# COMPiLELab/krylov_robustness

Hardware: AMD Instinct MI355X
Metric: trace(exp(A)) evals/sec + achieved HBM GB/s, n=1M nnz=10M, 1/2/4/8 GPU (higher is better)
Workload: dtype f64

## Files before the change

krylov_robustness_amd/csrc/kt_kernels.hip:

```cpp
#include <hip/hip_runtime.h>

#include "kt_launch.h"
#include "kt_wave.h"
#include <stdint.h>

#include <cstdlib>

#include <type_traits>

namespace kt {

__device__ __forceinline__ uint64_t sm64(uint64_t x) {
    uint64_t z = x + 0x9E3779B97F4A7C15ULL;
    z = (z ^ (z >> 30)) * 0xBF58476D1CE4E5B9ULL;
    z = (z ^ (z >> 27)) * 0x94D049BB133111EBULL;
    return z ^ (z >> 31);
}

template <int P, int VW> struct GeoW {
    static constexpr int VEC = VW;
    static constexpr int LPR = P / VEC;
    static constexpr int GPW = 64 / LPR;
};
template <int P> using Geo = GeoW<P, (P >= 2) ? 2 : 1>;
// ... 981 lines not shown
__global__ __launch_bounds__(256) void k_inf_norm(int n, int nc, const double* __restrict__ X,
                                                  int ldx, double* __restrict__ partial) {
    double mx = 0.0;
    for (int r = blockIdx.x * blockDim.x + threadIdx.x; r < n; r += gridDim.x * blockDim.x) {
        double s = 0.0;
        for (int c = 0; c < nc; ++c) s += fabs(X[(int64_t)r * ldx + c]);
        mx = fmax(mx, s);
    }
    for (int o = 32; o > 0; o >>= 1) mx = fmax(mx, kt::shfl_xor(mx, o));
    __shared__ double red[4];
    if ((threadIdx.x & 63) == 0) red[threadIdx.x >> 6] = mx;
    __syncthreads();
    if (threadIdx.x == 0) partial[blockIdx.x] = fmax(fmax(red[0], red[1]), fmax(red[2], red[3]));
}

__global__ __launch_bounds__(256) void k_normest1_y(int n, const double* __restrict__ Y,
                                                   const double* __restrict__ Sprev,
                                                   double* __restrict__ S,
                                                   double* __restrict__ partial) {
    double a = 0.0, d = 0.0;
    for (int r = blockIdx.x * blockDim.x + threadIdx.x; r < n; r += gridDim.x * blockDim.x) {
        const double y = Y[r];
        const double s = y < 0.0 ? -1.0 : 1.0;
        a += fabs(y);
        d = fma(Sprev[r], s, d);
        S[r] = s;
    }
    for (int o = 32; o > 0; o >>= 1) {
        a += kt::shfl_xor(a, o);
        d += kt::shfl_xor(d, o);
// ... 87 lines not shown
    if ((threadIdx.x & 63) == 0) red[threadIdx.x >> 6] = mx;
    __syncthreads();
    if (threadIdx.x == 0) {
        st->c1 = fmax(fmax(red[0], red[1]), fmax(red[2], red[3]));
        st->c1s[1] = st->c1;
        st->active = 1;
    }
    if (threadIdx.x < kTermSlots) {
        st->term_max[1][threadIdx.x][0] = 0ull;
        st->term_max[1][threadIdx.x][1] = 0ull;
    }
}

__global__ __launch_bounds__(256) void k_expmv_term(int n, int nc, double mu, double coef,
                                                    const double* __restrict__ Ab, double* __restrict__ b,
                                                    double* __restrict__ F, int ld,
                                                    double* __restrict__ partial,
                                                    const ExpmvState* __restrict__ st) {
    if (!st->active) return;
    double mb = 0.0, mf = 0.0;
    for (int r = blockIdx.x * blockDim.x + threadIdx.x; r < n; r += gridDim.x * blockDim.x) {
        double sb = 0.0, sf = 0.0;
        for (int c = 0; c < nc; ++c) {
            const int64_t o = (int64_t)r * ld + c;
            double t = Ab[o];
            if (mu != 0.0) t = fma(-mu, b[o], t);
            const double bn = fma(coef, t, 0.0);
            const double f = fma(1.0, bn, F[o]);
            b[o] = bn;
            F[o] = f;
            sb += fabs(bn);
            sf += fabs(f);
        }
        mb = fmax(mb, sb);
        mf = fmax(mf, sf);
    }
    for (int o = 32; o > 0; o >>= 1) {
        mb = fmax(mb, kt::shfl_xor(mb, o));
        mf = fmax(mf, kt::shfl_xor(mf, o));
    }
    __shared__ double red[2][4];
    if ((threadIdx.x & 63) == 0) {
        red[0][threadIdx.x >> 6] = mb;
        red[1][threadIdx.x >> 6] = mf;
    }
    __syncthreads();
    if (threadIdx.x == 0) {
        partial[blockIdx.x] = fmax(fmax(red[0][0], red[0][1]), fmax(red[0][2], red[0][3]));
        partial[gridDim.x + blockIdx.x] = fmax(fmax(red[1][0], red[1][1]), fmax(red[1][2], red[1][3]));
    }
}

template <int VEC>
__device__ __forceinline__ void expmv_row_prefetch(int row, int p0, int nc, int ld, double mu,
                                                   const double* __restrict__ bin,
                                                   const double* __restrict__ F, double* fo, double* bo) {
#pragma unroll
    for (int e = 0; e < VEC; ++e) {
        const int c = p0 + e;
        const int64_t o = (int64_t)row * ld + c;
        fo[e] = (c < nc) ? F[o] : 0.0;
        bo[e] = (c < nc && mu != 0.0) ? bin[o] : 0.0;
    }
}
template <int VEC, bool PADW = true>
__device__ __forceinline__ void expmv_row_update(int row, int p0, const double* s, const double* fo,
                                                 const double* bo, int nc, int ld, double mu, double coef,
                                                 double* __restrict__ bout, double* __restrict__ F,
                                                 double& sb, double& sf) {
#pragma unroll
    for (int e = 0; e < VEC; ++e) {
        const int c = p0 + e;
        const int64_t o = (int64_t)row * ld + c;
        if (c < nc) {
            double t = s[e];
            if (mu != 0.0) t = fma(-mu, bo[e], t);
            const double bn = fma(coef, t, 0.0);
            const double f = fma(1.0, bn, fo[e]);
            bout[o] = bn;
            F[o] = f;
            sb += fabs(bn);
            sf += fabs(f);
        } else if constexpr (PADW) {
            bout[o] = 0.0;
        }
    }
}

constexpr int kExpmvWaves = 4;
constexpr int kExpmvSplitBlocks = 1024;

template <int P, int FLAGS, bool SPLIT>
__global__ __launch_bounds__(64 * kExpmvWaves) void k_expmv_step(
    const int* __restrict__ rp, const int* __restrict__ ci, const double* __restrict__ va, int n,
    const int* __restrict__ long_rows, int n_long, const int* __restrict__ med_rows, int n_med,
    int nc, int ld, double mu, double coef, double tol, int k, const double* __restrict__ bin,
    double* __restrict__ bout, double* __restrict__ F, ExpmvState* st, int* hflag, int stage) {
    constexpr int WAVES = kExpmvWaves;
    using G = GeoW<P, (P >= 2) ? 2 : 1>;
    using GL = GeoW<P, (P >= 4) ? 4 : (P >= 2) ? 2 : 1>;
    __shared__ double red[2][WAVES];
    __shared__ double lred[WAVES][P];
    __shared__ int decide;
    const int lane = threadIdx.x & 63;
    const int wave = threadIdx.x >> 6;
    const int med_blocks = (n_med + WAVES - 1) / WAVES;
    const int kind = ((int)blockIdx.x < n_long) ? 2 : ((int)blockIdx.x < n_long + med_blocks) ? 1 : 0;
    if constexpr (SPLIT) {
        if (threadIdx.x == 0) decide = st->active;
        __syncthreads();
        if (!decide) return;
// ... 4 lines not shown
    if (!SPLIT && wave == 0 && k > 1) {
        pmb = st->term_max[(k - 1) % 3][lane][0];
        pmf = st->term_max[(k - 1) % 3][lane][1];
    }
    const int subL = lane % GL::LPR, grpL = lane / GL::LPR, p0L = subL * GL::VEC;
    const int sub = lane % G::LPR, grp = lane / G::LPR, p0 = sub * G::VEC;
    double sl[GL::VEC], s[G::VEC], fo[GL::VEC], bo[GL::VEC];
#pragma unroll
    for (int e = 0; e < GL::VEC; ++e) sl[e] = fo[e] = bo[e] = 0.0;
#pragma unroll
    for (int e = 0; e < G::VEC; ++e) s[e] = 0.0;
    int row = -1;
    bool mine = false;
    if (kind == 2) {
        row = long_rows[blockIdx.x];
        if (!SPLIT && wave == 0 && grpL == 0) expmv_row_prefetch<GL::VEC>(row, p0L, nc, ld, mu, bin, F, fo, bo);
        row_gather8<P, FLAGS, GL>(rp[row] + wave * GL::GPW + grpL, rp[row + 1], WAVES * GL::GPW, p0L, ci,
                                  va, bin, sl, ld);
    } else if (kind == 1) {
        const int mi = ((int)blockIdx.x - n_long) * WAVES + wave;
        if (mi < n_med) {
            row = med_rows[mi];
            if (!SPLIT && grpL == 0) expmv_row_prefetch<GL::VEC>(row, p0L, nc, ld, mu, bin, F, fo, bo);
            row_gather8<P, FLAGS, GL>(rp[row] + grpL, rp[row + 1], GL::GPW, p0L, ci, va, bin, sl, ld);
            mine = grpL == 0;
        }
    } else {
        row = (((int)blockIdx.x - n_long - med_blocks) * WAVES + wave) * G::GPW + grp;
        if (row < n) {
            const int beg = rp[row], end = rp[row + 1];
            if (end - beg <= kMedThresh) {
                if (!SPLIT) expmv_row_prefetch<G::VEC>(row, p0, nc, ld, mu, bin, F, fo, bo);
                row_gather8<P, FLAGS, G>(beg, end, 1, p0, ci, va, bin, s, ld);
                mine = true;
            }
        }
    }
    if (kind != 0) {
#pragma unroll
        for (int o = GL::LPR; o < 64; o <<= 1)
#pragma unroll
            for (int e = 0; e < GL::VEC; ++e) sl[e] += kt::shfl_xor(sl[e], o);
    }
    if (kind == 2 && grpL == 0)
#pragma unroll
        for (int e = 0; e < GL::VEC; ++e) lred[wave][p0L + e] = sl[e];
    if constexpr (!SPLIT) {
// ... 20 lines not shown
    __syncthreads();
    if (!decide) return;
    } else {
        __syncthreads();
    }
    if (blockIdx.x == 0) {
        if (threadIdx.x == 0) st->mv += 1;
        if (!SPLIT && threadIdx.x < kTermSlots) {
            st->term_max[(k + 1) % 3][threadIdx.x][0] = 0ull;
            st->term_max[(k + 1) % 3][threadIdx.x][1] = 0ull;
        }
    }
    double sb = 0.0, sf = 0.0;
    if (kind == 0) {
        if (mine) {
            if constexpr (SPLIT) expmv_row_prefetch<G::VEC>(row, p0, nc, ld, mu, bin, F, fo, bo);
            expmv_row_update<G::VEC>(row, p0, s, fo, bo, nc, ld, mu, coef, bout, F, sb, sf);
        }
#pragma unroll
        for (int o = 1; o < G::LPR; o <<= 1) {
            sb += kt::shfl_xor(sb, o);
            sf += kt::shfl_xor(sf, o);
        }
    } else {
        if (kind == 2 && wave == 0 && grpL == 0) {
#pragma unroll
            for (int e = 0; e < GL::VEC; ++e)
            {
                double t = lred[0][p0L + e];
#pragma unroll
                for (int w = 1; w < WAVES; ++w) t += lred[w][p0L + e];
                sl[e] = t;
            }
            mine = true;
        }
        if (mine) {
            if constexpr (SPLIT) expmv_row_prefetch<GL::VEC>(row, p0L, nc, ld, mu, bin, F, fo, bo);
            expmv_row_update<GL::VEC>(row, p0L, sl, fo, bo, nc, ld, mu, coef, bout, F, sb, sf);
        }
#pragma unroll
        for (int o = 1; o < GL::LPR; o <<= 1) {
            sb += kt::shfl_xor(sb, o);
            sf += kt::shfl_xor(sf, o);
        }
    }
    double mb = sb, mf = sf;
#pragma unroll
    for (int o = 32; o > 0; o >>= 1) {
        mb = fmax(mb, kt::shfl_xor(mb, o));
        mf = fmax(mf, kt::shfl_xor(mf, o));
    }
    if (lane == 0) {
        red[0][wave] = mb;
// ... 9 lines not shown
        }
        unsigned long long* slot = st->term_max[k % 3][blockIdx.x % kTermSlots];
        __hip_atomic_fetch_max(slot, (unsigned long long)__double_as_longlong(x), __ATOMIC_RELAXED,
                               __HIP_MEMORY_SCOPE_AGENT);
        __hip_atomic_fetch_max(slot + 1, (unsigned long long)__double_as_longlong(y), __ATOMIC_RELAXED,
                               __HIP_MEMORY_SCOPE_AGENT);
    }
}

constexpr int kExpmvRowsWaves = 4;
template <int P, int FLAGS, bool CHECK>
__global__ __launch_bounds__(64 * kExpmvRowsWaves) void k_expmv_rows(
    const int* __restrict__ rp, const int* __restrict__ ci, const double* __restrict__ va, int n,
    const int* __restrict__ long_rows, int n_long, int n_heavy, const int4* __restrict__ med_tasks, int n_med,
    const int4* __restrict__ short_tasks, int n_short,
    int nc, int ld, double mu, double coef, int k, const double* __restrict__ bin,
    double* __restrict__ bout, double* __restrict__ F, ExpmvState* st, double tol, int* hflag, int stage) {
    constexpr int WAVES = kExpmvRowsWaves;
    constexpr int VW = kExpmvWaves;
    using G = GeoW<P, (P >= 2) ? 2 : 1>;
    using GL = GeoW<P, (P >= 4) ? 4 : (P >= 2) ? 2 : 1>;
    constexpr bool MU0 = (FLAGS & KF_MU0) != 0;
    if constexpr (MU0) mu = 0.0;
    __shared__ int decide;
    __shared__ double red[2][WAVES];
    __shared__ double lsum[WAVES][P];
    const int lane = threadIdx.x & 63;
    const int wave = threadIdx.x >> 6;
    if (wave == 0) {
        int run = st->active;
        if (CHECK && k > 1 && run) {
// ... 55 lines not shown
            for (int e = 0; e < GL::VEC; ++e) acc[e] += kt::shfl_xor(acc[e], o);
        if (grpL == 0)
#pragma unroll
            for (int e = 0; e < GL::VEC; ++e) lsum[wave][p0L + e] = acc[e];
        __syncthreads();
        double sb = 0.0, sf = 0.0;
        if (wave == 0) {
            if (grpL == 0) {
                double t[GL::VEC], fo[GL::VEC], bo[GL::VEC];
#pragma unroll
                for (int e = 0; e < GL::VEC; ++e) {
                    t[e] = lsum[0][p0L + e];
#pragma unroll
                    for (int w = 1; w < VW; ++w) t[e] += lsum[w][p0L + e];
                }
                expmv_row_prefetch<GL::VEC>(row, p0L, nc, ld, mu, bin, F, fo, bo);
                expmv_row_update<GL::VEC, false>(row, p0L, t, fo, bo, nc, ld, mu, coef, bout, F, sb, sf);
            }
            fold(sb, sf, GL::LPR);
        }
        __syncthreads();
    }
    for (int li = n_heavy + gw; li < n_long; li += TW) {
        const int row = long_rows[li];
        const int beg = rp[row], end = rp[row + 1];
        double s[GL::VEC];
#pragma unroll 1
        for (int w = 0; w < VW; ++w) {
            double acc[GL::VEC];
#pragma unroll
            for (int e = 0; e < GL::VEC; ++e) acc[e] = 0.0;
            row_gather8<P, FLAGS, GL, 4>(beg + w * GL::GPW + grpL, end, VW * GL::GPW, p0L, ci, va, bin, acc, ld);
#pragma unroll
            for (int o = GL::LPR; o < 64; o <<= 1)
#pragma unroll
                for (int e = 0; e < GL::VEC; ++e) acc[e] += kt::shfl_xor(acc[e], o);
#pragma unroll
            for (int e = 0; e < GL::VEC; ++e) s[e] = w == 0 ? acc[e] : s[e] + acc[e];
        }
        double sb = 0.0, sf = 0.0;
        if (grpL == 0) {
            double fo[GL::VEC], bo[GL::VEC];
            expmv_row_prefetch<GL::VEC>(row, p0L, nc, ld, mu, bin, F, fo, bo);
            expmv_row_update<GL::VEC, false>(row, p0L, s, fo, bo, nc, ld, mu, coef, bout, F, sb, sf);
        }
        fold(sb, sf, GL::LPR);
    }
    constexpr int MD = 4;
    auto load_mtask = [&](int ii, int& r, int& bg, int& en) {
        r = -1;
        bg = en = 0;
        if (ii < n_med) {
            const int4 v = med_tasks[ii];
            r = v.x;
            bg = v.y;
            en = v.z;
        }
    };
    auto load_mchunk = [&](int bg, int en, int* c) {
        const int k0 = bg + grpL;
        const int c0 = k0 < en ? ld_stream<FLAGS>(ci + k0) : 0;
        c[0] = c0;
#pragma unroll
        for (int i = 1; i < MD; ++i) c[i] = (k0 + i * GL::GPW < en) ? ld_stream<FLAGS>(ci + k0 + i * GL::GPW) : c0;
    };
    {
        auto load_mf = [&](int r, double* f) {
#pragma unroll
            for (int e = 0; e < GL::VEC; ++e) {
                const int c = p0L + e;
                f[e] = (MU0 && grpL == 0 && r >= 0 && c < nc) ? F[(int64_t)r * ld + c] : 0.0;
            }
        };
        int mi = gw;
        int row, beg, end, nrow, nbeg, nend;
        load_mtask(mi, row, beg, end);
        int mc[MD];
        load_mchunk(beg, end, mc);
        double mfc[GL::VEC];
        load_mf(row, mfc);
        load_mtask(mi + TW, nrow, nbeg, nend);
        for (; mi < n_med; mi += TW) {
            int nnrow, nnbeg, nnend;
            load_mtask(mi + 2 * TW, nnrow, nnbeg, nnend);
            int mn[MD];
            load_mchunk(nbeg, nend, mn);
            double mfn[GL::VEC];
// ... 22 lines not shown
                        else s[e] = fma(a[i], VL::get(x[i], e), s[e]);
                    }
            }
            row_gather8<P, FLAGS, GL, MD>(k0 + MD * GL::GPW, end, GL::GPW, p0L, ci, va, bin, s, ld);
#pragma unroll
            for (int o = GL::LPR; o < 64; o <<= 1)
#pragma unroll
                for (int e = 0; e < GL::VEC; ++e) s[e] += kt::shfl_xor(s[e], o);
            double sb = 0.0, sf = 0.0;
            if (grpL == 0) {
                double fo[GL::VEC], bo[GL::VEC];
                if constexpr (MU0) {
#pragma unroll
                    for (int e = 0; e < GL::VEC; ++e) fo[e] = mfc[e];
                } else {
                    expmv_row_prefetch<GL::VEC>(row, p0L, nc, ld, mu, bin, F, fo, bo);
                }
                expmv_row_update<GL::VEC, false>(row, p0L, s, fo, bo, nc, ld, mu, coef, bout, F, sb, sf);
            }
            fold(sb, sf, GL::LPR);
#pragma unroll
            for (int e = 0; e < GL::VEC; ++e) mfc[e] = mfn[e];
            row = nrow;
            beg = nbeg;
            end = nend;
            nrow = nnrow;
            nbeg = nnbeg;
            nend = nnend;
#pragma unroll
            for (int i = 0; i < MD; ++i) mc[i] = mn[i];
        }
    }
    constexpr int SD = 8;
// ... 4 lines not shown
        r = -1;
        bg = en = 0;
        if (bb < nblk && t < n_short) {
            const int4 v = short_tasks[t];
            r = v.x;
            bg = v.y;
            en = v.z;
        }
    };
    auto load_chunk = [&](int bg, int en, int* c) {
        const int c0 = bg < en ? ld_stream<FLAGS>(ci + bg) : 0;
        c[0] = c0;
#pragma unroll
        for (int i = 1; i < SCOL; ++i) c[i] = (bg + i < en) ? ld_stream<FLAGS>(ci + bg + i) : c0;
    };
    auto load_f = [&](int r, double* f) {
#pragma unroll
        for (int e = 0; e < G::VEC; ++e) {
            const int c = p0 + e;
            f[e] = (MU0 && r >= 0 && c < nc) ? F[(int64_t)r * ld + c] : 0.0;
        }
    };
    int b = gw;
    int row, beg, end, nrow, nbeg, nend;
    load_task(b, row, beg, end);
    int cc[SCOL];
    load_chunk(beg, end, cc);
    double fc[G::VEC];
    load_f(row, fc);
    load_task(b + TW, nrow, nbeg, nend);
    for (; b < nblk; b += TW) {
        int nnrow, nnbeg, nnend;
        load_task(b + 2 * TW, nnrow, nnbeg, nnend);
        int cn[SCOL];
        load_chunk(nbeg, nend, cn);
        double fn[G::VEC];
        load_f(nrow, fn);
// ... 16 lines not shown
#pragma unroll
                for (int i = 0; i < SD; ++i) x[i] = VV::load(bin + (int64_t)cc[h * SD + i] * ld + p0);
#pragma unroll
                for (int i = 0; i < SD; ++i)
#pragma unroll
                    for (int e = 0; e < G::VEC; ++e) {
                        if constexpr (FLAGS & KF_UNIT) s[e] = (k0 + i < end) ? s[e] + VV::get(x[i], e) : s[e];
                        else s[e] = fma(a[i], VV::get(x[i], e), s[e]);
                    }
            }
            row_gather8<P, FLAGS, G, SD>(beg + SCOL, end, 1, p0, ci, va, bin, s, ld);
            if constexpr (MU0) {
#pragma unroll
                for (int e = 0; e < G::VEC; ++e) fo[e] = fc[e];
            } else {
                expmv_row_prefetch<G::VEC>(row, p0, nc, ld, mu, bin, F, fo, bo);
            }
            expmv_row_update<G::VEC, false>(row, p0, s, fo, bo, nc, ld, mu, coef, bout, F, sb, sf);
        }
        fold(sb, sf, G::LPR);
#pragma unroll
        for (int e = 0; e < G::VEC; ++e) fc[e] = fn[e];
        row = nrow;
        beg = nbeg;
        end = nend;
        nrow = nnrow;
        nbeg = nnbeg;
        nend = nnend;
#pragma unroll
        for (int i = 0; i < SCOL; ++i) cc[i] = cn[i];
    }
#pragma unroll
    for (int o = 32; o > 0; o >>= 1) {
// ... 318 lines not shown

hipError_t launch_axpby(int n, int nc, double a, const double* X, int ldx, double b, double* Y,
                        int ldy, hipStream_t st) {
    k_axpby<<<stream_grid((int64_t)n * nc), 256, 0, st>>>(n, nc, a, X, ldx, b, Y, ldy);
    return hipGetLastError();
}

int inf_norm_blocks() { return 1024; }

hipError_t launch_inf_norm(int n, int nc, const double* X, int ldx, double* partial,
                           hipStream_t st) {
    k_inf_norm<<<inf_norm_blocks(), 256, 0, st>>>(n, nc, X, ldx, partial);
    return hipGetLastError();
}

static int expmv_term_blocks(int n) {
    const int b = (n + 255) / 256;
    return b < 1 ? 1 : (b > inf_norm_blocks() ? inf_norm_blocks() : b);
}

hipError_t launch_expmv_begin(const double* partial, int nb, void* state, hipStream_t st) {
    k_expmv_begin<<<1, 256, 0, st>>>(partial, nb, static_cast<ExpmvState*>(state));
    return hipGetLastError();
}

hipError_t launch_expmv_term(int n, int nc, double mu, double coef, const double* Ab, double* b,
                             double* F, int ld, double* partial, const void* state, hipStream_t st) {
    k_expmv_term<<<expmv_term_blocks(n), 256, 0, st>>>(n, nc, mu, coef, Ab, b, F, ld, partial,
                                                       static_cast<const ExpmvState*>(state));
    return hipGetLastError();
}

hipError_t launch_expmv_check(int n, const double* partial, double tol, void* state, hipStream_t st) {
    k_expmv_check<<<1, 256, 0, st>>>(partial, expmv_term_blocks(n), tol, static_cast<ExpmvState*>(state));
    return hipGetLastError();
}

size_t expmv_state_bytes() { return sizeof(ExpmvState); }

int expmv_step_blocks(int n, int P, int n_long, int n_med, int waves) {
    if (waves <= 0) waves = kExpmvWaves;
    const int gpw = (P >= 2) ? 64 / (P / 2) : 64;
    return n_long + (n_med + waves - 1) / waves + (n + waves * gpw - 1) / (waves * gpw);
// ... 11 lines not shown
static int expmv_rows_grid(int n_tasks_hint) {
    static const int resident = [] {
        int dev = 0, cus = 0, occ = 0;
        (void)hipGetDevice(&dev);
        (void)hipDeviceGetAttribute(&cus, hipDeviceAttributeMultiprocessorCount, dev);
        (void)hipOccupancyMaxActiveBlocksPerMultiprocessor(&occ, k_expmv_rows<16, KF_UNIT | KF_MU0, true>,
                                                           64 * kExpmvRowsWaves, 0);
        return (occ > 0 ? occ : 2) * (cus > 0 ? cus : 256);
    }();
    int g = resident;
    if (g > n_tasks_hint) g = n_tasks_hint;
    return g < 1 ? 1 : g;
}

hipError_t launch_expmv_step(int P, bool unit, const CsrView& M, const int* med_rows, int n_med, int nc,
                             int ld, double mu, double coef, double tol, int k, const double* bin,
                             double* bout, double* F, void* state, hipStream_t st, int form, int* hflag,
                             int stage) {
    ExpmvState* s = static_cast<ExpmvState*>(state);
    if ((form == 2 || form == 3) && !(M.short_tasks && M.med_tasks)) form = 1;
    if (form == 2 || form == 3) {
        const bool fused_check = form == 3;
        static const int classes = [] {
            const char* e = std::getenv("KT_EXPMV_CLASSES");
            return e ? std::atoi(e) : 7;
        }();
        const int nl = (classes & 1) ? M.n_long : 0, nh = (classes & 1) ? M.n_heavy : 0, nm = (classes & 2) ? n_med : 0,
                  ns = (classes & 4) ? M.n_short : 0;
        const int tasks = nl + nm + (ns + 7) / 8;
        const int grid = expmv_rows_grid((tasks + kExpmvRowsWaves - 1) / kExpmvRowsWaves);
#define KT_EXPMV_ROWS(PP, F_)                                                                      \
    if (fused_check)                                                                               \
        k_expmv_rows<PP, F_, true><<<grid, 64 * kExpmvRowsWaves, 0, st>>>(M.rp, M.ci, M.va, M.n, M.long_rows, \
            nl, nh, reinterpret_cast<const int4*>(M.med_tasks), nm, reinterpret_cast<const int4*>(M.short_tasks), \
            ns, nc, ld, mu, coef, k, bin, bout, F, s, tol, hflag, stage);                          \
    else                                                                                           \
        k_expmv_rows<PP, F_, false><<<grid, 64 * kExpmvRowsWaves, 0, st>>>(M.rp, M.ci, M.va, M.n, M.long_rows, \
            nl, nh, reinterpret_cast<const int4*>(M.med_tasks), nm, reinterpret_cast<const int4*>(M.short_tasks), \
            ns, nc, ld, mu, coef, k, bin, bout, F, s, tol, hflag, stage)
#define KT_EXPMV_ROWS_P(PP)                                                                        \
    if (mu == 0.0) {                                                                               \
        if (unit) KT_EXPMV_ROWS(PP, KF_UNIT | KF_MU0);                                             \
        else KT_EXPMV_ROWS(PP, KF_MU0);                                                            \
    } else {                                                                                       \
        if (unit) KT_EXPMV_ROWS(PP, KF_UNIT);                                                      \
        else KT_EXPMV_ROWS(PP, 0);                                                                 \
    }
        switch (P) {
        case 1: KT_EXPMV_ROWS_P(1) break;
        case 2: KT_EXPMV_ROWS_P(2) break;
        case 4: KT_EXPMV_ROWS_P(4) break;
        case 8: KT_EXPMV_ROWS_P(8) break;
        case 16: KT_EXPMV_ROWS_P(16) break;
        case 32: KT_EXPMV_ROWS_P(32) break;
        default: return hipErrorInvalidValue;
        }
#undef KT_EXPMV_ROWS_P
#undef KT_EXPMV_ROWS
        return hipGetLastError();
    }
    const bool split = form == 1;
    const int grid = expmv_step_blocks(M.n, P, M.n_long, n_med);
#define KT_EXPMV_LAUNCH(PP, F_, SP)                                                                \
    k_expmv_step<PP, F_, SP><<<grid, 64 * kExpmvWaves, 0, st>>>(M.rp, M.ci, M.va, M.n, M.long_rows, \
                                                               M.n_long, med_rows, n_med, nc, ld, mu, \
                                                               coef, tol, k, bin, bout, F, s, hflag, stage)
#define KT_EXPMV_STEP(PP)                                                                          \
    if (unit) {                                                                                    \
        if (split) KT_EXPMV_LAUNCH(PP, KF_UNIT, true);                                             \
        else KT_EXPMV_LAUNCH(PP, KF_UNIT, false);                                                  \
    } else {                                                                                       \
        if (split) KT_EXPMV_LAUNCH(PP, 0, true);                                                   \
        else KT_EXPMV_LAUNCH(PP, 0, false);                                                        \
    }
    switch (P) {
    case 1: KT_EXPMV_STEP(1) break;
    case 2: KT_EXPMV_STEP(2) break;
    case 4: KT_EXPMV_STEP(4) break;
    case 8: KT_EXPMV_STEP(8) break;
    case 16: KT_EXPMV_STEP(16) break;
// ... 94 lines not shown
```

krylov_robustness_amd/csrc/kt_launch.h:

```cpp
#pragma once
#include <hip/hip_runtime.h>
#include <stdint.h>

namespace kt {

int spmm_grid(int n, int P, int max_blocks);
int long_blocks_for(int n_long, int max_blocks);

hipError_t launch_rademacher(int P, int n, uint64_t seed, int64_t probe_base, const int* perm,
                             double* X, hipStream_t st);
hipError_t launch_rademacher_cols(int n, int ncols, uint64_t seed, int64_t probe_base, double* X, int ldx,
                                  hipStream_t st);
hipError_t launch_spmm_dot(int P, int flags, int grid, const int* rp, const int* ci,
                           const double* va, int n, const double* ucur, const double* sc,
                           double* y, double* partial, const int* long_rows, int n_long,
                           int long_thresh, int long_blocks, hipStream_t st);
struct CsrView {
    const int* rp;
    const int* ci;
    const double* va;
    int n;
    const int* long_rows;
    int n_long, long_thresh, split_thresh;
    const int* ck_beg;
// ... 107 lines not shown
                        int batch = 1);
int col_nrb(int n, int num_cu, int rpb_lo = 64);
hipError_t launch_col_dots(int n, int P, int nb, int64_t vstride, const double* V, const double* W,
                           int r_lo, int num_cu, double* part, double* out, hipStream_t st, int rpb_lo = 64);
hipError_t launch_col_update(int n, int P, int nb, int64_t vstride, const double* V,
                             const double* h, double* W, hipStream_t st);
hipError_t launch_col_householder(int n, int P, const double* s, double* W, double* Q, double* r,
                                  hipStream_t st);
hipError_t launch_col_select(int C, int P, const int* idx, double* X, hipStream_t st);
size_t pairs_coef_doubles(int C);
hipError_t launch_inf_norm(int n, int nc, const double* X, int ldx, double* partial,
                           hipStream_t st);
size_t expmv_state_bytes();
hipError_t launch_expmv_begin(const double* partial, int nb, void* state, hipStream_t st);
hipError_t launch_expmv_term(int n, int nc, double mu, double coef, const double* Ab, double* b,
                             double* F, int ld, double* partial, const void* state, hipStream_t st);
hipError_t launch_expmv_check(int n, const double* partial, double tol, void* state, hipStream_t st);
int expmv_step_blocks(int n, int P, int n_long, int n_med, int waves = 0);
bool expmv_split_check(int n, int P, int n_long, int n_med);
hipError_t launch_expmv_slot_check(void* state, int k, double tol, hipStream_t st, int* hflag, int stage);
hipError_t launch_expmv_step(int P, bool unit, const CsrView& M, const int* med_rows, int n_med, int nc,
                             int ld, double mu, double coef,
                             double tol, int k, const double* bin, double* bout, double* F,
                             void* state, hipStream_t st, int form, int* hflag = nullptr, int stage = 0);

}
```

krylov_robustness_amd/csrc/kt_mctrace.cpp:

```cpp
#include <algorithm>
#include <cmath>
#include <cstdio>
#include <cstdlib>
#include <thread>

#include "kt_krylov.h"
#include "kt_worker.h"
#include "kt_launch.h"
#include "kt_slq.h"

namespace kt {

static const double kTheta[100] = {
2.2204460492503131e-16, 2.5809568029946243e-08, 1.3863478661191185e-05, 0.00033971688399768305,
0.0024008763578872742, 0.0090656564075951018, 0.023844555325002736, 0.049912288711153226,
0.08957760203223343, 0.1441829761614378, 0.21423580684517107, 0.29961589138115802,
0.3997775336316795, 0.51391469361242936, 0.64108352330411988, 0.78028742566265763,
0.93053284607865683, 1.0908637192900361, 1.2603810606426387, 1.4382525968043369,
1.6237159502358214, 1.8160778162150852, 2.0147107809446161, 2.2190488693650896,
2.4285825244428265, 2.6428534574594353, 2.8614496339342641, 3.0840005449891619,
3.3101728398902708, 3.5396663487436895, 3.772210495681751, 4.0075610861180397,
4.2454974425796959, 4.4858198594473686, 4.728347345793539, 4.9729156261919814,
5.219375371084058, 5.4675906305245441, 5.7174374475720127, 5.9688026300418491,
6.221582661689891, 6.4756827360799845, 6.731015898381024, 6.9875022821306301,
// ... 133 lines not shown
                imax = hi[b];
            }
        if (k >= 2 && hmax == std::fabs(zbest)) break;
        ind = imax;
        unit(X.col(0), ind);
        std::swap(S, S_old);
        ++k;
    }
    return {est, it2 * m};
}

struct Expmv {
    int s = 1, m = 0, mv = 0;
};

static Expmv expmv_device(kt_matrix_s* A, double t, const double* Bsrc, int ld, int nc, double* F) {
    kt_context_s* ctx = A->ctx;
    const int64_t n = A->n;
    hipStream_t st = ctx->stream;
    Expmv r;
    ctx->expmv_calls += 1;
    if (A->expmv_sel_ok && A->expmv_sel_version == A->version && A->expmv_sel_t == t &&
        A->expmv_sel_nc == nc) {
        r.s = A->expmv_sel_s;
        r.m = A->expmv_sel_m;
        r.mv = A->expmv_sel_mv;
    } else {
        double trA = 0.0;
        for (int64_t i = 0; i < n; ++i)
            for (int64_t k = A->h_rowptr[i]; k < A->h_rowptr[i + 1]; ++k)
                if (A->h_col[k] == i) trA += A->h_val[k];
// ... 60 lines not shown
        if (cost == INFINITY) cost = 0.0;
        r.m = m_best;
        r.s = (int)std::max(cost / std::max(m_best, 1), 1.0);
        A->expmv_sel_ok = true;
        A->expmv_sel_version = A->version;
        A->expmv_sel_t = t;
        A->expmv_sel_nc = nc;
        A->expmv_sel_mu = mu;
        A->expmv_sel_s = r.s;
        A->expmv_sel_m = r.m;
        A->expmv_sel_mv = r.mv;
    }
    const double mu = A->expmv_sel_mu;
    const double tol = std::ldexp(1.0, -53);
    const double eta = std::exp(t * mu / r.s);
    DevMat b, Ab;
    b.alloc(ctx, n, ld);
    Ab.alloc(ctx, n, ld);
    copy_cols(ctx, n, Bsrc, ld, b.col(0), ld, nc);
    copy_cols(ctx, n, Bsrc, ld, F, ld, nc);
    const int nb = inf_norm_blocks();
    ctx->ws.norm_part.ensure(sizeof(double) * 2 * nb);
    ctx->ws.expmv_state.ensure(expmv_state_bytes());
    double* part = ctx->ws.norm_part.as<double>();
    void* state = ctx->ws.expmv_state.ptr;
    KT_HIP(hipMemsetAsync(state, 0, expmv_state_bytes(), st));
    const int P = pow2_at_least(std::max(nc, 1));
    if (P <= 32 && ld >= P && !std::getenv("KT_EXPMV_UNFUSED")) {
        const DevCSR& M0 = natural_csr(A);
        const char* spe = std::getenv("KT_EXPMV_SPLIT");
        const bool split = spe ? spe[0] == '1' : expmv_split_check((int)n, P, M0.n_long, M0.n_med);
        const char* rwe = std::getenv("KT_EXPMV_ROWS");
        const char* rce = std::getenv("KT_EXPMV_ROWCHECK");
        int form = !split ? 0 : (rwe && rwe[0] == '0') ? 1 : (rce && rce[0] == '0') ? 2 : 3;
        if (form >= 2 && !(M0.short_tasks && M0.med_tasks)) form = 1;
        const DevCSR& M = M0;
        const CsrView V{M.rowptr, M.col, M.val, (int)n, M.long_rows, M.n_long, A->long_thresh,
                        kSplitThresh, M.ck_beg, M.ck_end, M.n_chunks, M.sp_rows, M.sp_first, M.n_split,
                        M.short_tasks, M.n_short, M.med_tasks, M.n_heavy};
        const char* sf = std::getenv("KT_EXPMV_STOPFLAG");
// ... 4 lines not shown
            __atomic_store_n(ctx->ws.expmv_stop.host, -1, __ATOMIC_RELEASE);
            hflag = ctx->ws.expmv_stop.dev;
        }
        const int ahead = (split && use_flag) ? 3 : 0;
        std::vector<hipEvent_t> ring(ahead, nullptr);
        for (auto& e : ring) KT_HIP(hipEventCreateWithFlags(&e, hipEventDisableTiming));
        struct RingGuard {
            std::vector<hipEvent_t>& r;
            ~RingGuard() {
                for (hipEvent_t e : r)
                    if (e) (void)hipEventDestroy(e);
            }
        } ring_guard{ring};
        int64_t queued = 0;
        for (int i = 0; i < r.s; ++i) {
            KT_HIP(launch_inf_norm((int)n, nc, b.col(0), ld, part, st));
            KT_HIP(launch_expmv_begin(part, nb, state, st));
            double* cur = b.col(0);
            double* nxt = Ab.col(0);
            for (int k = 1; k <= r.m; ++k) {
                if (ahead && queued >= ahead) KT_HIP(hipEventSynchronize(ring[queued % ahead]));
                if (use_flag && k > 2 && __atomic_load_n(ctx->ws.expmv_stop.host, __ATOMIC_ACQUIRE) >= i) break;
                prof_begin(ctx, PROF_EXPMV, st, form);
                KT_HIP(launch_expmv_step(P, A->unit_values, V, M.med_rows, M.n_med, nc, ld, mu,
                                         t / ((double)r.s * k), tol, k, cur, nxt, F, state, st, form, hflag, i));
                prof_end(ctx, PROF_EXPMV, st);
                if ((form == 1 || form == 2) && k < r.m) KT_HIP(launch_expmv_slot_check(state, k, tol, st, hflag, i));
                if (ahead) KT_HIP(hipEventRecord(ring[queued % ahead], st));
                ++queued;
                std::swap(cur, nxt);
            }
            KT_HIP(launch_axpby((int)n, nc, eta, F, ld, 0.0, F, ld, st));
            copy_cols(ctx, n, F, ld, b.col(0), ld, nc);
        }
        int hstate[2] = {0, 0};
        KT_HIP(hipMemcpyAsync(hstate, state, sizeof(hstate), hipMemcpyDeviceToHost, st));
        KT_HIP(hipStreamSynchronize(st));
        r.mv += hstate[1];
        ctx->expmv_terms += hstate[1];
        return r;
    }
    for (int i = 0; i < r.s; ++i) {
        KT_HIP(launch_inf_norm((int)n, nc, b.col(0), ld, part, st));
        KT_HIP(launch_expmv_begin(part, nb, state, st));
        for (int k = 1; k <= r.m; ++k) {
            spmm_slices(A, b.col(0), ld, Ab.col(0), ld, nc, static_cast<const int*>(state));
            KT_HIP(launch_expmv_term((int)n, nc, mu, t / ((double)r.s * k), Ab.col(0), b.col(0), F, ld,
                                     part, state, st));
            KT_HIP(launch_expmv_check((int)n, part, tol, state, st));
        }
        KT_HIP(launch_axpby((int)n, nc, eta, F, ld, 0.0, F, ld, st));
        copy_cols(ctx, n, F, ld, b.col(0), ld, nc);
    }
    int hstate[2] = {0, 0};
    KT_HIP(hipMemcpyAsync(hstate, state, sizeof(hstate), hipMemcpyDeviceToHost, st));
    KT_HIP(hipStreamSynchronize(st));
    r.mv += hstate[1];
    ctx->expmv_terms += hstate[1];
    return r;
}

struct AfunDev {
    kt_matrix_s* A;
    int kind, fun, m;
    void apply(const double* X, int ld, int nc, double* Y) {
        switch (kind) {
        case AFUN_MATRIX: spmm(A, X, ld, Y, ld, nc); break;
// ... 377 lines not shown
```

Before: 2.611.

## Fuse expmv stage-end scale, copy and inf-norm; compact F accumulator stride

Adds a stage-end kernel that scales F by eta, writes it back and into the next-stage b (or the output), and computes the row-wise inf-norm partials in the same pass. This replaces the separate axpby, copy_cols and inf_norm launches at every stage and the two initial copies. F now lives in a private buffer with a compact leading dimension (nc rounded to even) instead of ld, which cuts F traffic in the step kernels. The cost is an extra allocation and a final copy into the caller's output, plus an ldf parameter threaded through every expmv kernel.

```diff
diff --git a/krylov_robustness_amd/csrc/kt_kernels.hip b/krylov_robustness_amd/csrc/kt_kernels.hip
--- a/krylov_robustness_amd/csrc/kt_kernels.hip
+++ b/krylov_robustness_amd/csrc/kt_kernels.hip
@@ -1019,6 +1019,46 @@
     if (threadIdx.x == 0) partial[blockIdx.x] = fmax(fmax(red[0], red[1]), fmax(red[2], red[3]));
 }
 
+template <bool SCALE, bool PAIR>
+__global__ __launch_bounds__(256) void k_expmv_stage_end(int n, int nc, double eta, const double* src, int lds,
+                                                         double* Fw, int ldf, double* dst, int ldd,
+                                                         double* __restrict__ partial) {
+    double mx = 0.0;
+    for (int r = blockIdx.x * blockDim.x + threadIdx.x; r < n; r += gridDim.x * blockDim.x) {
+        const double* ps = src + (int64_t)r * lds;
+        double* pf = Fw ? Fw + (int64_t)r * ldf : nullptr;
+        double* pd = dst + (int64_t)r * ldd;
+        double s = 0.0;
+        int c = 0;
+        if constexpr (PAIR) {
+            for (; c + 1 < nc; c += 2) {
+                double2 v = *reinterpret_cast<const double2*>(ps + c);
+                if constexpr (SCALE) {
+                    v.x = fma(eta, v.x, 0.0);
+                    v.y = fma(eta, v.y, 0.0);
+                }
+                if (pf) *reinterpret_cast<double2*>(pf + c) = v;
+                *reinterpret_cast<double2*>(pd + c) = v;
+                s += fabs(v.x);
+                s += fabs(v.y);
+            }
+        }
+        for (; c < nc; ++c) {
+            double x = ps[c];
+            if constexpr (SCALE) x = fma(eta, x, 0.0);
+            if (pf) pf[c] = x;
+            pd[c] = x;
+            s += fabs(x);
+        }
+        mx = fmax(mx, s);
+    }
+    for (int o = 32; o > 0; o >>= 1) mx = fmax(mx, kt::shfl_xor(mx, o));
+    __shared__ double red[4];
+    if ((threadIdx.x & 63) == 0) red[threadIdx.x >> 6] = mx;
+    __syncthreads();
+    if (threadIdx.x == 0) partial[blockIdx.x] = fmax(fmax(red[0], red[1]), fmax(red[2], red[3]));
+}
+
 __global__ __launch_bounds__(256) void k_normest1_y(int n, const double* __restrict__ Y,
                                                    const double* __restrict__ Sprev,
                                                    double* __restrict__ S,
@@ -1136,7 +1176,7 @@
 
 __global__ __launch_bounds__(256) void k_expmv_term(int n, int nc, double mu, double coef,
                                                     const double* __restrict__ Ab, double* __restrict__ b,
-                                                    double* __restrict__ F, int ld,
+                                                    double* __restrict__ F, int ld, int ldf,
                                                     double* __restrict__ partial,
                                                     const ExpmvState* __restrict__ st) {
     if (!st->active) return;
@@ -1144,13 +1184,13 @@
     for (int r = blockIdx.x * blockDim.x + threadIdx.x; r < n; r += gridDim.x * blockDim.x) {
         double sb = 0.0, sf = 0.0;
         for (int c = 0; c < nc; ++c) {
-            const int64_t o = (int64_t)r * ld + c;
+            const int64_t o = (int64_t)r * ld + c, of = (int64_t)r * ldf + c;
             double t = Ab[o];
             if (mu != 0.0) t = fma(-mu, b[o], t);
             const double bn = fma(coef, t, 0.0);
-            const double f = fma(1.0, bn, F[o]);
+            const double f = fma(1.0, bn, F[of]);
             b[o] = bn;
-            F[o] = f;
+            F[of] = f;
             sb += fabs(bn);
             sf += fabs(f);
         }
@@ -1174,20 +1214,28 @@
 }
 
 template <int VEC>
-__device__ __forceinline__ void expmv_row_prefetch(int row, int p0, int nc, int ld, double mu,
+__device__ __forceinline__ void expmv_load_f(int row, int p0, int nc, int ldf, bool live,
+                                             const double* __restrict__ F, double* f) {
+#pragma unroll
+    for (int e = 0; e < VEC; ++e) {
+        const int c = p0 + e;
+        f[e] = (live && c < nc) ? F[(int64_t)row * ldf + c] : 0.0;
+    }
+}
+template <int VEC>
+__device__ __forceinline__ void expmv_row_prefetch(int row, int p0, int nc, int ld, int ldf, double mu,
                                                    const double* __restrict__ bin,
                                                    const double* __restrict__ F, double* fo, double* bo) {
+    expmv_load_f<VEC>(row, p0, nc, ldf, true, F, fo);
 #pragma unroll
     for (int e = 0; e < VEC; ++e) {
         const int c = p0 + e;
-        const int64_t o = (int64_t)row * ld + c;
-        fo[e] = (c < nc) ? F[o] : 0.0;
-        bo[e] = (c < nc && mu != 0.0) ? bin[o] : 0.0;
+        bo[e] = (c < nc && mu != 0.0) ? bin[(int64_t)row * ld + c] : 0.0;
     }
 }
 template <int VEC, bool PADW = true>
 __device__ __forceinline__ void expmv_row_update(int row, int p0, const double* s, const double* fo,
-                                                 const double* bo, int nc, int ld, double mu, double coef,
+                                                 const double* bo, int nc, int ld, int ldf, double mu, double coef,
                                                  double* __restrict__ bout, double* __restrict__ F,
                                                  double& sb, double& sf) {
 #pragma unroll
@@ -1200,7 +1248,7 @@
             const double bn = fma(coef, t, 0.0);
             const double f = fma(1.0, bn, fo[e]);
             bout[o] = bn;
-            F[o] = f;
+            F[(int64_t)row * ldf + c] = f;
             sb += fabs(bn);
             sf += fabs(f);
         } else if constexpr (PADW) {
@@ -1216,7 +1264,7 @@
 __global__ __launch_bounds__(64 * kExpmvWaves) void k_expmv_step(
     const int* __restrict__ rp, const int* __restrict__ ci, const double* __restrict__ va, int n,
     const int* __restrict__ long_rows, int n_long, const int* __restrict__ med_rows, int n_med,
-    int nc, int ld, double mu, double coef, double tol, int k, const double* __restrict__ bin,
+    int nc, int ld, int ldf, double mu, double coef, double tol, int k, const double* __restrict__ bin,
     double* __restrict__ bout, double* __restrict__ F, ExpmvState* st, int* hflag, int stage) {
     constexpr int WAVES = kExpmvWaves;
     using G = GeoW<P, (P >= 2) ? 2 : 1>;
@@ -1251,14 +1299,14 @@
     bool mine = false;
     if (kind == 2) {
         row = long_rows[blockIdx.x];
-        if (!SPLIT && wave == 0 && grpL == 0) expmv_row_prefetch<GL::VEC>(row, p0L, nc, ld, mu, bin, F, fo, bo);
+        if (!SPLIT && wave == 0 && grpL == 0) expmv_row_prefetch<GL::VEC>(row, p0L, nc, ld, ldf, mu, bin, F, fo, bo);
         row_gather8<P, FLAGS, GL>(rp[row] + wave * GL::GPW + grpL, rp[row + 1], WAVES * GL::GPW, p0L, ci,
                                   va, bin, sl, ld);
     } else if (kind == 1) {
         const int mi = ((int)blockIdx.x - n_long) * WAVES + wave;
         if (mi < n_med) {
             row = med_rows[mi];
-            if (!SPLIT && grpL == 0) expmv_row_prefetch<GL::VEC>(row, p0L, nc, ld, mu, bin, F, fo, bo);
+            if (!SPLIT && grpL == 0) expmv_row_prefetch<GL::VEC>(row, p0L, nc, ld, ldf, mu, bin, F, fo, bo);
             row_gather8<P, FLAGS, GL>(rp[row] + grpL, rp[row + 1], GL::GPW, p0L, ci, va, bin, sl, ld);
             mine = grpL == 0;
         }
@@ -1267,7 +1315,7 @@
         if (row < n) {
             const int beg = rp[row], end = rp[row + 1];
             if (end - beg <= kMedThresh) {
-                if (!SPLIT) expmv_row_prefetch<G::VEC>(row, p0, nc, ld, mu, bin, F, fo, bo);
+                if (!SPLIT) expmv_row_prefetch<G::VEC>(row, p0, nc, ld, ldf, mu, bin, F, fo, bo);
                 row_gather8<P, FLAGS, G>(beg, end, 1, p0, ci, va, bin, s, ld);
                 mine = true;
             }
@@ -1318,8 +1366,8 @@
     double sb = 0.0, sf = 0.0;
     if (kind == 0) {
         if (mine) {
-            if constexpr (SPLIT) expmv_row_prefetch<G::VEC>(row, p0, nc, ld, mu, bin, F, fo, bo);
-            expmv_row_update<G::VEC>(row, p0, s, fo, bo, nc, ld, mu, coef, bout, F, sb, sf);
+            if constexpr (SPLIT) expmv_row_prefetch<G::VEC>(row, p0, nc, ld, ldf, mu, bin, F, fo, bo);
+            expmv_row_update<G::VEC>(row, p0, s, fo, bo, nc, ld, ldf, mu, coef, bout, F, sb, sf);
         }
 #pragma unroll
         for (int o = 1; o < G::LPR; o <<= 1) {
@@ -1339,8 +1387,8 @@
             mine = true;
         }
         if (mine) {
-            if constexpr (SPLIT) expmv_row_prefetch<GL::VEC>(row, p0L, nc, ld, mu, bin, F, fo, bo);
-            expmv_row_update<GL::VEC>(row, p0L, sl, fo, bo, nc, ld, mu, coef, bout, F, sb, sf);
+            if constexpr (SPLIT) expmv_row_prefetch<GL::VEC>(row, p0L, nc, ld, ldf, mu, bin, F, fo, bo);
+            expmv_row_update<GL::VEC>(row, p0L, sl, fo, bo, nc, ld, ldf, mu, coef, bout, F, sb, sf);
         }
 #pragma unroll
         for (int o = 1; o < GL::LPR; o <<= 1) {
@@ -1380,7 +1428,7 @@
     const int* __restrict__ rp, const int* __restrict__ ci, const double* __restrict__ va, int n,
     const int* __restrict__ long_rows, int n_long, int n_heavy, const int4* __restrict__ med_tasks, int n_med,
     const int4* __restrict__ short_tasks, int n_short,
-    int nc, int ld, double mu, double coef, int k, const double* __restrict__ bin,
+    int nc, int ld, int ldf, double mu, double coef, int k, const double* __restrict__ bin,
     double* __restrict__ bout, double* __restrict__ F, ExpmvState* st, double tol, int* hflag, int stage) {
     constexpr int WAVES = kExpmvRowsWaves;
     constexpr int VW = kExpmvWaves;
@@ -1466,8 +1514,8 @@
 #pragma unroll
                     for (int w = 1; w < VW; ++w) t[e] += lsum[w][p0L + e];
                 }
-                expmv_row_prefetch<GL::VEC>(row, p0L, nc, ld, mu, bin, F, fo, bo);
-                expmv_row_update<GL::VEC, false>(row, p0L, t, fo, bo, nc, ld, mu, coef, bout, F, sb, sf);
+                expmv_row_prefetch<GL::VEC>(row, p0L, nc, ld, ldf, mu, bin, F, fo, bo);
+                expmv_row_update<GL::VEC, false>(row, p0L, t, fo, bo, nc, ld, ldf, mu, coef, bout, F, sb, sf);
             }
             fold(sb, sf, GL::LPR);
         }
@@ -1493,8 +1541,8 @@
         double sb = 0.0, sf = 0.0;
         if (grpL == 0) {
             double fo[GL::VEC], bo[GL::VEC];
-            expmv_row_prefetch<GL::VEC>(row, p0L, nc, ld, mu, bin, F, fo, bo);
-            expmv_row_update<GL::VEC, false>(row, p0L, s, fo, bo, nc, ld, mu, coef, bout, F, sb, sf);
+            expmv_row_prefetch<GL::VEC>(row, p0L, nc, ld, ldf, mu, bin, F, fo, bo);
+            expmv_row_update<GL::VEC, false>(row, p0L, s, fo, bo, nc, ld, ldf, mu, coef, bout, F, sb, sf);
         }
         fold(sb, sf, GL::LPR);
     }
@@ -1518,11 +1566,7 @@
     };
     {
         auto load_mf = [&](int r, double* f) {
-#pragma unroll
-            for (int e = 0; e < GL::VEC; ++e) {
-                const int c = p0L + e;
-                f[e] = (MU0 && grpL == 0 && r >= 0 && c < nc) ? F[(int64_t)r * ld + c] : 0.0;
-            }
+            expmv_load_f<GL::VEC>(r, p0L, nc, ldf, MU0 && grpL == 0 && r >= 0, F, f);
         };
         int mi = gw;
         int row, beg, end, nrow, nbeg, nend;
@@ -1575,9 +1619,9 @@
 #pragma unroll
                     for (int e = 0; e < GL::VEC; ++e) fo[e] = mfc[e];
                 } else {
-                    expmv_row_prefetch<GL::VEC>(row, p0L, nc, ld, mu, bin, F, fo, bo);
+                    expmv_row_prefetch<GL::VEC>(row, p0L, nc, ld, ldf, mu, bin, F, fo, bo);
                 }
-                expmv_row_update<GL::VEC, false>(row, p0L, s, fo, bo, nc, ld, mu, coef, bout, F, sb, sf);
+                expmv_row_update<GL::VEC, false>(row, p0L, s, fo, bo, nc, ld, ldf, mu, coef, bout, F, sb, sf);
             }
             fold(sb, sf, GL::LPR);
 #pragma unroll
@@ -1612,13 +1656,7 @@
 #pragma unroll
         for (int i = 1; i < SCOL; ++i) c[i] = (bg + i < en) ? ld_stream<FLAGS>(ci + bg + i) : c0;
     };
-    auto load_f = [&](int r, double* f) {
-#pragma unroll
-        for (int e = 0; e < G::VEC; ++e) {
-            const int c = p0 + e;
-            f[e] = (MU0 && r >= 0 && c < nc) ? F[(int64_t)r * ld + c] : 0.0;
-        }
-    };
+    auto load_f = [&](int r, double* f) { expmv_load_f<G::VEC>(r, p0, nc, ldf, MU0 && r >= 0, F, f); };
     int b = gw;
     int row, beg, end, nrow, nbeg, nend;
     load_task(b, row, beg, end);
@@ -1665,9 +1703,9 @@
 #pragma unroll
                 for (int e = 0; e < G::VEC; ++e) fo[e] = fc[e];
             } else {
-                expmv_row_prefetch<G::VEC>(row, p0, nc, ld, mu, bin, F, fo, bo);
+                expmv_row_prefetch<G::VEC>(row, p0, nc, ld, ldf, mu, bin, F, fo, bo);
             }
-            expmv_row_update<G::VEC, false>(row, p0, s, fo, bo, nc, ld, mu, coef, bout, F, sb, sf);
+            expmv_row_update<G::VEC, false>(row, p0, s, fo, bo, nc, ld, ldf, mu, coef, bout, F, sb, sf);
         }
         fold(sb, sf, G::LPR);
 #pragma unroll
@@ -2016,6 +2054,24 @@
     return hipGetLastError();
 }
 
+hipError_t launch_expmv_stage_end(int n, int nc, double eta, bool scale, const double* src, int lds, double* Fw,
+                                  int ldf, double* dst, int ldd, double* partial, hipStream_t st) {
+    const bool pair = ((lds | ldf | ldd) & 1) == 0 &&
+                      ((reinterpret_cast<uintptr_t>(src) | reinterpret_cast<uintptr_t>(Fw) |
+                        reinterpret_cast<uintptr_t>(dst)) & 15) == 0;
+#define KT_STAGE_END(SC, PR) \
+    k_expmv_stage_end<SC, PR><<<inf_norm_blocks(), 256, 0, st>>>(n, nc, eta, src, lds, Fw, ldf, dst, ldd, partial)
+    if (scale) {
+        if (pair) KT_STAGE_END(true, true);
+        else KT_STAGE_END(true, false);
+    } else {
+        if (pair) KT_STAGE_END(false, true);
+        else KT_STAGE_END(false, false);
+    }
+#undef KT_STAGE_END
+    return hipGetLastError();
+}
+
 static int expmv_term_blocks(int n) {
     const int b = (n + 255) / 256;
     return b < 1 ? 1 : (b > inf_norm_blocks() ? inf_norm_blocks() : b);
@@ -2027,8 +2083,8 @@
 }
 
 hipError_t launch_expmv_term(int n, int nc, double mu, double coef, const double* Ab, double* b,
-                             double* F, int ld, double* partial, const void* state, hipStream_t st) {
-    k_expmv_term<<<expmv_term_blocks(n), 256, 0, st>>>(n, nc, mu, coef, Ab, b, F, ld, partial,
+                             double* F, int ld, int ldf, double* partial, const void* state, hipStream_t st) {
+    k_expmv_term<<<expmv_term_blocks(n), 256, 0, st>>>(n, nc, mu, coef, Ab, b, F, ld, ldf, partial,
                                                        static_cast<const ExpmvState*>(state));
     return hipGetLastError();
 }
@@ -2070,7 +2126,7 @@
 }
 
 hipError_t launch_expmv_step(int P, bool unit, const CsrView& M, const int* med_rows, int n_med, int nc,
-                             int ld, double mu, double coef, double tol, int k, const double* bin,
+                             int ld, int ldf, double mu, double coef, double tol, int k, const double* bin,
                              double* bout, double* F, void* state, hipStream_t st, int form, int* hflag,
                              int stage) {
     ExpmvState* s = static_cast<ExpmvState*>(state);
@@ -2089,11 +2145,11 @@
     if (fused_check)                                                                               \
         k_expmv_rows<PP, F_, true><<<grid, 64 * kExpmvRowsWaves, 0, st>>>(M.rp, M.ci, M.va, M.n, M.long_rows, \
             nl, nh, reinterpret_cast<const int4*>(M.med_tasks), nm, reinterpret_cast<const int4*>(M.short_tasks), \
-            ns, nc, ld, mu, coef, k, bin, bout, F, s, tol, hflag, stage);                          \
+            ns, nc, ld, ldf, mu, coef, k, bin, bout, F, s, tol, hflag, stage);                          \
     else                                                                                           \
         k_expmv_rows<PP, F_, false><<<grid, 64 * kExpmvRowsWaves, 0, st>>>(M.rp, M.ci, M.va, M.n, M.long_rows, \
             nl, nh, reinterpret_cast<const int4*>(M.med_tasks), nm, reinterpret_cast<const int4*>(M.short_tasks), \
-            ns, nc, ld, mu, coef, k, bin, bout, F, s, tol, hflag, stage)
+            ns, nc, ld, ldf, mu, coef, k, bin, bout, F, s, tol, hflag, stage)
 #define KT_EXPMV_ROWS_P(PP)                                                                        \
     if (mu == 0.0) {                                                                               \
         if (unit) KT_EXPMV_ROWS(PP, KF_UNIT | KF_MU0);                                             \
@@ -2119,7 +2175,7 @@
     const int grid = expmv_step_blocks(M.n, P, M.n_long, n_med);
 #define KT_EXPMV_LAUNCH(PP, F_, SP)                                                                \
     k_expmv_step<PP, F_, SP><<<grid, 64 * kExpmvWaves, 0, st>>>(M.rp, M.ci, M.va, M.n, M.long_rows, \
-                                                               M.n_long, med_rows, n_med, nc, ld, mu, \
+                                                               M.n_long, med_rows, n_med, nc, ld, ldf, mu, \
                                                                coef, tol, k, bin, bout, F, s, hflag, stage)
 #define KT_EXPMV_STEP(PP)                                                                          \
     if (unit) {                                                                                    \
diff --git a/krylov_robustness_amd/csrc/kt_launch.h b/krylov_robustness_amd/csrc/kt_launch.h
--- a/krylov_robustness_amd/csrc/kt_launch.h
+++ b/krylov_robustness_amd/csrc/kt_launch.h
@@ -145,13 +145,15 @@
 size_t expmv_state_bytes();
 hipError_t launch_expmv_begin(const double* partial, int nb, void* state, hipStream_t st);
 hipError_t launch_expmv_term(int n, int nc, double mu, double coef, const double* Ab, double* b,
-                             double* F, int ld, double* partial, const void* state, hipStream_t st);
+                             double* F, int ld, int ldf, double* partial, const void* state, hipStream_t st);
+hipError_t launch_expmv_stage_end(int n, int nc, double eta, bool scale, const double* src, int lds, double* Fw,
+                                  int ldf, double* dst, int ldd, double* partial, hipStream_t st);
 hipError_t launch_expmv_check(int n, const double* partial, double tol, void* state, hipStream_t st);
 int expmv_step_blocks(int n, int P, int n_long, int n_med, int waves = 0);
 bool expmv_split_check(int n, int P, int n_long, int n_med);
 hipError_t launch_expmv_slot_check(void* state, int k, double tol, hipStream_t st, int* hflag, int stage);
 hipError_t launch_expmv_step(int P, bool unit, const CsrView& M, const int* med_rows, int n_med, int nc,
-                             int ld, double mu, double coef,
+                             int ld, int ldf, double mu, double coef,
                              double tol, int k, const double* bin, double* bout, double* F,
                              void* state, hipStream_t st, int form, int* hflag = nullptr, int stage = 0);
 
diff --git a/krylov_robustness_amd/csrc/kt_mctrace.cpp b/krylov_robustness_amd/csrc/kt_mctrace.cpp
--- a/krylov_robustness_amd/csrc/kt_mctrace.cpp
+++ b/krylov_robustness_amd/csrc/kt_mctrace.cpp
@@ -171,7 +171,7 @@
     int s = 1, m = 0, mv = 0;
 };
 
-static Expmv expmv_device(kt_matrix_s* A, double t, const double* Bsrc, int ld, int nc, double* F) {
+static Expmv expmv_device(kt_matrix_s* A, double t, const double* Bsrc, int ld, int nc, double* Fout) {
     kt_context_s* ctx = A->ctx;
     const int64_t n = A->n;
     hipStream_t st = ctx->stream;
@@ -262,16 +262,26 @@
     const double mu = A->expmv_sel_mu;
     const double tol = std::ldexp(1.0, -53);
     const double eta = std::exp(t * mu / r.s);
-    DevMat b, Ab;
+    const int ldf = std::min(ld, (nc + 1) & ~1);
+    DevMat b, Ab, Fc;
     b.alloc(ctx, n, ld);
     Ab.alloc(ctx, n, ld);
-    copy_cols(ctx, n, Bsrc, ld, b.col(0), ld, nc);
-    copy_cols(ctx, n, Bsrc, ld, F, ld, nc);
+    Fc.alloc(ctx, n, ldf, false);
+    double* F = Fc.col(0);
+    const bool scale = eta != 1.0 || r.m == 0;
     const int nb = inf_norm_blocks();
     ctx->ws.norm_part.ensure(sizeof(double) * 2 * nb);
     ctx->ws.expmv_state.ensure(expmv_state_bytes());
     double* part = ctx->ws.norm_part.as<double>();
     void* state = ctx->ws.expmv_state.ptr;
+    KT_HIP(launch_expmv_stage_end((int)n, nc, 1.0, false, Bsrc, ld, F, ldf, b.col(0), ld, part, st));
+    auto stage_end = [&](int i) {
+        if (i + 1 < r.s)
+            KT_HIP(launch_expmv_stage_end((int)n, nc, eta, scale, F, ldf, scale ? F : nullptr, ldf, b.col(0), ld,
+                                          part, st));
+        else
+            KT_HIP(launch_expmv_stage_end((int)n, nc, eta, scale, F, ldf, nullptr, ldf, Fout, ld, part, st));
+    };
     KT_HIP(hipMemsetAsync(state, 0, expmv_state_bytes(), st));
     const int P = pow2_at_least(std::max(nc, 1));
     if (P <= 32 && ld >= P && !std::getenv("KT_EXPMV_UNFUSED")) {
@@ -306,7 +316,6 @@
         } ring_guard{ring};
         int64_t queued = 0;
         for (int i = 0; i < r.s; ++i) {
-            KT_HIP(launch_inf_norm((int)n, nc, b.col(0), ld, part, st));
             KT_HIP(launch_expmv_begin(part, nb, state, st));
             double* cur = b.col(0);
             double* nxt = Ab.col(0);
@@ -314,7 +323,7 @@
                 if (ahead && queued >= ahead) KT_HIP(hipEventSynchronize(ring[queued % ahead]));
                 if (use_flag && k > 2 && __atomic_load_n(ctx->ws.expmv_stop.host, __ATOMIC_ACQUIRE) >= i) break;
                 prof_begin(ctx, PROF_EXPMV, st, form);
-                KT_HIP(launch_expmv_step(P, A->unit_values, V, M.med_rows, M.n_med, nc, ld, mu,
+                KT_HIP(launch_expmv_step(P, A->unit_values, V, M.med_rows, M.n_med, nc, ld, ldf, mu,
                                          t / ((double)r.s * k), tol, k, cur, nxt, F, state, st, form, hflag, i));
                 prof_end(ctx, PROF_EXPMV, st);
                 if ((form == 1 || form == 2) && k < r.m) KT_HIP(launch_expmv_slot_check(state, k, tol, st, hflag, i));
@@ -322,8 +331,7 @@
                 ++queued;
                 std::swap(cur, nxt);
             }
-            KT_HIP(launch_axpby((int)n, nc, eta, F, ld, 0.0, F, ld, st));
-            copy_cols(ctx, n, F, ld, b.col(0), ld, nc);
+            stage_end(i);
         }
         int hstate[2] = {0, 0};
         KT_HIP(hipMemcpyAsync(hstate, state, sizeof(hstate), hipMemcpyDeviceToHost, st));
@@ -333,16 +341,14 @@
         return r;
     }
     for (int i = 0; i < r.s; ++i) {
-        KT_HIP(launch_inf_norm((int)n, nc, b.col(0), ld, part, st));
         KT_HIP(launch_expmv_begin(part, nb, state, st));
         for (int k = 1; k <= r.m; ++k) {
             spmm_slices(A, b.col(0), ld, Ab.col(0), ld, nc, static_cast<const int*>(state));
             KT_HIP(launch_expmv_term((int)n, nc, mu, t / ((double)r.s * k), Ab.col(0), b.col(0), F, ld,
-                                     part, state, st));
+                                     ldf, part, state, st));
             KT_HIP(launch_expmv_check((int)n, part, tol, state, st));
         }
-        KT_HIP(launch_axpby((int)n, nc, eta, F, ld, 0.0, F, ld, st));
-        copy_cols(ctx, n, F, ld, b.col(0), ld, nc);
+        stage_end(i);
     }
     int hstate[2] = {0, 0};
     KT_HIP(hipMemcpyAsync(hstate, state, sizeof(hstate), hipMemcpyDeviceToHost, st));
```

New measurement: 2.610. About the same (-0.1%).
